# abeauvisage/uasl_motion_estimation

Hardware: AMD Instinct MI355X
Metric: frames/sec + BA iter/sec, 2000 feats x 20-keyframe window, 1/2/4/8 MI355X (higher is better)
Workload: dtype u8+f32 (MI), f64 (BA); 1 GPU; config 3: 1280x720 stereo, 2000 feats, 20-keyframe window, 11x11 MI patches; frame=KLT + MI scale LM (LM, MAX_NB_ITER 10, tolerances off) + 10 BA LM iterations, parallelism=1 independent streams (one per GPU)

## Files before the change

include/me_hip.h:

```cpp
#ifndef ME_HIP_H
#define ME_HIP_H
#include <stddef.h>
#include <stdint.h>

#ifdef __cplusplus
extern "C" {
#endif

#define ME_ABI_VERSION 4

enum {
  ME_OK = 0,
  ME_ERR_INVALID = -1,
  ME_ERR_HIP = -2,
  ME_ERR_NOMEM = -3,
  ME_ERR_UNSUPPORTED = -4,
  ME_ERR_STATE = -5,
  ME_ERR_NO_DEVICE = -6
};

typedef enum { ME_HOST = 0, ME_DEVICE = 1 } me_mem;

typedef struct me_ctx me_ctx;

// ... 124 lines not shown
  double function_tolerance;
  double gradient_tolerance;
  double parameter_tolerance;
  double initial_trust_region_radius, max_trust_region_radius, min_trust_region_radius;
  double min_lm_diagonal, max_lm_diagonal, min_relative_decrease;
  int max_num_consecutive_invalid_steps;
  int jacobi_scaling;
} me_ba_options;

typedef struct {
  int status;
  int termination;
  int iterations;
  int successful_steps;
  double initial_cost, final_cost;
} me_ba_summary;

void me_ba_default_options(me_ba_options* o);
int me_ba_solve(me_ctx* ctx, me_ba_problem* p, const me_ba_options* o, me_ba_summary* s);
int me_ba_solve_async(me_ctx* ctx, me_ba_problem* p, const me_ba_options* o);
int me_ba_wait(me_ctx* ctx, me_ba_summary* s);
int me_ba_wait_out(me_ctx* ctx, me_ba_summary* s, double* cams, double* pts);
int me_ba_reserve(me_ctx* ctx, int n_cams, int n_pts, int n_obs, int obs_dim, int fixed_frames);
typedef struct me_vo_chain_args {
  double pose[6];
  double R[9];
  double vel[6];
  int k1, k0, mode;
} me_vo_chain_args;
int me_vo_ba_chain(me_ctx* ctx, double* cams, int n_cams, double* pts, int n_pts, const int32_t* cam_src,
                   const int32_t* win_ids, const int32_t* prev_ids, int n_prev, int32_t new_from,
                   const me_vo_chain_args* a);
typedef struct me_vo_window {
  const void* stage;
  void* dev;
  size_t stage_bytes;
  int chain;
  const int32_t* cam_src;
  const int32_t* win_ids;
  const int32_t* prev_ids;
  int n_prev;
  int32_t new_from;
  me_vo_chain_args args;
  const int32_t* frame;
  const int32_t* ids;
  int first_frame;
// ... 222 lines not shown
```

uasl_motion_estimation_amd/_lib.py:

```python
from __future__ import annotations

import ctypes
import os
from ctypes import POINTER, c_double, c_float, c_int, c_int32, c_long, c_size_t, c_uint8, c_uint32, c_void_p

import numpy as np

try:
    import torch
except Exception:
    torch = None

_HERE = os.path.dirname(os.path.abspath(__file__))
LIB_PATH = os.path.join(_HERE, "libme_hip.so")

ME_OK = 0
ME_HOST = 0
ME_DEVICE = 1
ERRORS = {
    -1: "ME_ERR_INVALID",
    -2: "ME_ERR_HIP",
    -3: "ME_ERR_NOMEM",
    -4: "ME_ERR_UNSUPPORTED",
    -5: "ME_ERR_STATE",
# ... 139 lines not shown
                ("n_usable", ctypes.c_int32), ("n_inliers", ctypes.c_int32), ("steps", ctypes.c_int32),
                ("valid", ctypes.c_int32), ("R", c_double * 9), ("t_rel", c_double * 3)]


class ClaheParamsC(ctypes.Structure):
    _fields_ = [("tiles_x", c_int), ("tiles_y", c_int), ("clip_limit", c_double)]


class ToneMapParamsC(ctypes.Structure):
    _fields_ = [("lo_ppm", c_int), ("hi_ppm", c_int), ("min_span", c_int), ("alpha_q8", c_int)]


ALLREDUCE_FN = ctypes.CFUNCTYPE(c_int, POINTER(c_double), c_int, c_void_p)

EXPORTS = [
    "me_abi_version", "me_range_push", "me_range_pop", "me_device_count", "me_create", "me_destroy", "me_last_error", "me_set_stream",
    "me_get_stream", "me_set_cu_mask", "me_stream_flags", "me_cu_count", "me_synchronize", "me_malloc", "me_free", "me_memcpy_h2d", "me_memcpy_d2h", "me_memcpy_d2d",
    "me_memcpy_async", "me_host_alloc", "me_host_free", "me_hbm_copy_gbs",
    "me_timing_enable", "me_timing_read", "me_timing_reset", "me_timing_sample",
    "me_mi_scores", "me_mutual_information", "me_entropy", "me_mi_epipolar_match", "me_mi_epipolar_match_count", "me_mi_epipolar_match_lr", "me_mi_epipolar_match_lr_count", "me_vo_new_cells", "me_compare_pc", "me_ccoeff_normed", "me_quantise",
    "me_optim_default_params", "me_scale_residuals", "me_scale_normal_equations", "me_scale_jacobian",
    "me_scale_optimise", "me_scale_last_counters", "me_scale_persistent", "me_scale_state_mi", "me_scale_inliers",
    "me_ba_default_options", "me_ba_solve", "me_ba_cost", "me_ba_evaluate", "me_ba_reduced_system",
    "me_ba_solve_sharded", "me_ba_covariance", "me_ba_solve_async", "me_ba_wait", "me_ba_wait_out", "me_ba_reserve", "me_ba_window_indices",
    "me_vo_ba_chain", "me_vo_window_submit",
    "me_comm_unique_id", "me_comm_create_rccl", "me_comm_create_callback", "me_comm_destroy", "me_comm_info",
    "me_comm_allreduce", "me_comm_calibrate", "me_comm_exchange_us", "me_ba_shard_worthwhile_comm", "me_ba_solve_comm", "me_ba_shard_worthwhile", "me_ba_shard_exchange_us",
    "me_klt_default_params", "me_klt_track", "me_klt_track_fb", "me_klt_track_guided", "me_klt_track_guided_fb",
    "me_corner_default_params", "me_corner_response", "me_vo_new_corners",
    "me_rectify_map", "me_remap_tile_dims", "me_remap_q5", "me_vo_loop_set_rectify",
    "me_clahe_default_params", "me_clahe", "me_clahe_apply_rows", "me_vo_loop_set_equalise",
    "me_tonemap_default_params", "me_tonemap_state_create", "me_tonemap_state_destroy", "me_tonemap_state_reset",
    "me_tonemap_state_read", "me_tonemap16", "me_vo_loop_set_tonemap", "me_vo_loop_process16",
    "me_nms_scanline3x3",
    "me_vo_default_params", "me_vo_srand", "me_vo_rand", "me_vo_process",
    "me_mono_default_params", "me_mono_vo_process",
    "me_vo_loop_default_config", "me_vo_loop_create", "me_vo_loop_destroy", "me_vo_loop_last_error",
    "me_vo_loop_process", "me_vo_loop_finish", "me_vo_loop_results", "me_vo_loop_events", "me_vo_loop_tracks",
    "me_vo_loop_poses", "me_vo_loop_frame_obs", "me_vo_loop_frames", "me_vo_loop_stats", "me_vo_loop_set_match_lr",
    "me_motion_gate_default_params", "me_motion_gate", "me_vo_loop_set_motion_gate",
    "me_vo_loop_set_klt_predict",
    "me_kf_default_params", "me_kf_update", "me_vo_loop_set_keyframe_select", "me_vo_loop_push",
    "me_frame_pose_default_params", "me_frame_pose", "me_vo_loop_set_frame_pose", "me_vo_loop_frame_poses",
]

class MonoParamsC(ctypes.Structure):
    _fields_ = [("fu", c_double), ("fv", c_double), ("cu", c_double), ("cv", c_double), ("prob", c_double),
# ... 60 lines not shown
                                               c_void_p, c_void_p, c_int, c_int, c_int, c_int, c_int, c_double,
                                               c_float, c_void_p, c_void_p]),
        "me_mi_epipolar_match_lr": (c_int, [c_void_p, c_void_p, c_void_p, c_int, c_int, c_int, c_void_p, c_void_p,
                                            c_void_p, c_void_p, c_int, c_int, c_int, c_int, c_int, c_double, c_float,
                                            c_double, c_void_p, c_void_p, c_void_p]),
        "me_mi_epipolar_match_lr_count": (c_int, [c_void_p, c_void_p, c_void_p, c_int, c_int, c_int, c_void_p,
                                                  c_void_p, c_void_p, c_int, c_int, c_int, c_int, c_int, c_double,
                                                  c_float, c_double, c_void_p, c_void_p, c_void_p]),
        "me_vo_new_cells": (c_int, [c_void_p, c_void_p, c_void_p, c_void_p, c_int, c_int, c_int, c_float, c_int, c_int,
                                    c_double, c_double, c_int, c_int, c_int, c_void_p, c_void_p, c_void_p]),
        "me_compare_pc": (c_int, [c_void_p, c_int, c_void_p, c_void_p, c_int, c_int, c_int, c_void_p]),
        "me_ccoeff_normed": (c_int, [c_void_p, c_int, c_void_p, c_void_p, c_int, c_int, c_int, c_void_p]),
        "me_quantise": (c_int, [c_void_p, c_int, c_void_p, c_int, c_int, c_int, c_int, c_int]),
        "me_entropy": (c_int, [c_void_p, c_int, c_void_p, c_int, c_int, c_int, c_void_p]),
        "me_optim_default_params": (None, [P(OptimParamsC)]),
        "me_scale_residuals": (c_int, [c_void_p, P(ScaleStateC), c_int, P(c_double), P(c_int)]),
        "me_scale_normal_equations": (c_int, [c_void_p, P(ScaleStateC), c_int, P(c_double), P(c_double),
                                              P(c_double)]),
        "me_scale_jacobian": (c_int, [c_void_p, P(ScaleStateC), c_int, P(c_double)]),
        "me_scale_optimise": (c_int, [c_void_p, P(ScaleStateC), P(OptimParamsC), c_int, P(c_int), P(c_int),
                                      P(c_double), c_int, P(c_long)]),
        "me_scale_last_counters": (c_int, [c_void_p, P(c_long), P(c_long), P(c_long), P(c_long)]),
        "me_scale_persistent": (c_int, [c_int, c_int]),
        "me_scale_state_mi": (c_int, [c_void_p, P(ScaleStateC), P(c_double), P(c_int)]),
        "me_scale_inliers": (c_int, [c_void_p, P(ScaleStateC), c_int, c_double, P(c_int), c_int, P(c_int)]),
        "me_ba_default_options": (None, [P(BAOptionsC)]),
        "me_ba_solve": (c_int, [c_void_p, P(BAProblemC), P(BAOptionsC), P(BASummaryC)]),
        "me_ba_solve_async": (c_int, [c_void_p, P(BAProblemC), P(BAOptionsC)]),
        "me_ba_wait": (c_int, [c_void_p, P(BASummaryC)]),
        "me_ba_wait_out": (c_int, [c_void_p, P(BASummaryC), c_void_p, c_void_p]),
        "me_ba_reserve": (c_int, [c_void_p, c_int, c_int, c_int, c_int, c_int]),
        "me_vo_window_submit": (c_int, [c_void_p, P(VOWindowC), P(BAProblemC), P(BAOptionsC)]),
        "me_vo_ba_chain": (c_int, [c_void_p, c_void_p, c_int, c_void_p, c_int, c_void_p, c_void_p, c_void_p, c_int,
                                   ctypes.c_int32, P(VOChainArgsC)]),
        "me_ba_cost": (c_int, [c_void_p, P(BAProblemC), P(c_double)]),
        "me_ba_window_indices": (c_int, [c_void_p, c_void_p, c_void_p, c_int, c_int, c_void_p, c_int, c_void_p,
                                         c_void_p]),
        "me_ba_evaluate": (c_int, [c_void_p, P(BAProblemC), P(c_double), P(c_double), P(c_double)]),
        "me_ba_reduced_system": (c_int, [c_void_p, P(BAProblemC), c_double, P(c_double), P(c_double)]),
        "me_ba_covariance": (c_int, [c_void_p, P(BAProblemC), P(c_double), P(c_int)]),
        "me_ba_solve_sharded": (c_int, [c_void_p, P(BAProblemC), P(BAOptionsC), ALLREDUCE_FN, c_void_p,
                                        P(BASummaryC)]),
        "me_comm_unique_id": (c_int, [c_void_p, c_int]),
        "me_comm_create_rccl": (c_int, [c_void_p, c_int, c_int, c_void_p, P(c_void_p)]),
        "me_comm_create_callback": (c_int, [c_void_p, c_int, c_int, ALLREDUCE_FN, c_void_p, P(c_void_p)]),
        "me_comm_destroy": (None, [c_void_p]),
# ... 61 lines not shown
        "me_vo_loop_set_frame_pose": (c_int, [c_void_p, P(FramePoseParamsC)]),
        "me_vo_loop_frame_poses": (c_int, [c_void_p, P(VoFramePoseC), c_int, P(c_int)]),
        "me_tonemap_default_params": (None, [P(ToneMapParamsC)]),
        "me_tonemap_state_create": (c_int, [c_void_p, P(c_void_p)]),
        "me_tonemap_state_destroy": (c_int, [c_void_p]),
        "me_tonemap_state_reset": (c_int, [c_void_p]),
        "me_tonemap_state_read": (c_int, [c_void_p, P(ctypes.c_int32)]),
        "me_tonemap16": (c_int, [c_void_p, c_int, c_void_p, c_int, c_int, c_int, c_void_p, c_int, P(ToneMapParamsC),
                                 c_void_p]),
        "me_vo_loop_set_tonemap": (c_int, [c_void_p, P(ToneMapParamsC)]),
        "me_vo_loop_process16": (c_int, [c_void_p, c_int, c_void_p, c_void_p, c_int]),
        "me_nms_scanline3x3": (c_int, [c_void_p, c_int, c_void_p, c_int, c_int, c_void_p, c_void_p, c_int,
                                       P(c_int)]),
        "me_vo_default_params": (None, [P(VOParamsC)]),
        "me_vo_srand": (c_int, [c_void_p, ctypes.c_uint]),
        "me_vo_rand": (c_int, [c_void_p, P(c_int)]),
        "me_vo_process": (c_int, [c_void_p, c_void_p, c_int, P(c_double), P(VOParamsC), c_int, P(c_double),
                                  P(c_double), P(c_double), P(c_int), P(c_int), P(c_int)]),
        "me_mono_default_params": (None, [P(MonoParamsC)]),
        "me_mono_vo_process": (c_int, [c_void_p, c_void_p, c_void_p, c_int, P(MonoParamsC), P(c_double),
                                       P(c_double), c_void_p, P(c_int), P(c_int)]),
    }
    for name, (res, args) in sig.items():
        fn = getattr(lib, name)
        fn.restype = res
        fn.argtypes = args
    _lib = lib
    return lib


def dptr(a: np.ndarray, ctype=c_double):
    if a is None:
        return None
    assert a.flags["C_CONTIGUOUS"], "array must be C-contiguous"
    return a.ctypes.data_as(POINTER(ctype))


def vptr(a):
    if a is None:
        return None
    if isinstance(a, int):
        return c_void_p(a)
    assert a.flags["C_CONTIGUOUS"], "array must be C-contiguous"
    return c_void_p(a.ctypes.data)


def cu_split(ncu: int, front_of_16: int, mode: str | None = None):
# ... 141 lines not shown
```

uasl_motion_estimation_amd/csrc/ba.hip:

```cpp
#include <algorithm>
#include <cmath>
#include <cstdio>
#include <cstring>
#include <mutex>
#include <numeric>
#include <vector>
#include <hip/hip_ext.h>
#include "me_internal.hpp"
#include "ba_kernels.hpp"
#include "roster.hpp"
#include "solve_diag.hpp"
#include "me_device.hpp"

using me_dev::wave_sync;

using namespace ba;

namespace {

constexpr double kDblMin = 2.2250738585072014e-308;
constexpr double kDblEps = 2.220446049250313e-16;

template <int Ctrl>
__device__ __forceinline__ double dpp_f64(double x);
// ... 2727 lines not shown
  }
  __syncthreads();
  for (int p = t; p < g.npairs; p += kScanBlock) {
    int I = 0, rem = p;
    while (rem >= g.T - I) {
      rem -= g.T - I;
      ++I;
    }
    const int J = I + rem;
    int cnt = 0;
    for (int r = 0; r < g.nruns; ++r) {
      const int A = rA[r], B = rB[r];
      const int nb = B - A + 1, ns = nb + (B < g.T - 1 ? 1 : 0);
      const int ka = (I >= A && I <= B) ? I - A : (I == g.T - 1 ? nb : -1);
      const int kb = (J >= A && J <= B) ? J - A : (J == g.T - 1 ? nb : -1);
      if (ka < 0 || kb < 0) continue;
      b.tl[(long)p * g.nruns + cnt++] = r * g.npairs + ka * ns - ka * (ka - 1) / 2 + (kb - ka);
    }
    b.tcnt[p] = cnt;
    for (int q = cnt; q < g.nruns; ++q) b.tl[(long)p * g.nruns + q] = -1;
  }
}

__global__ __launch_bounds__(kBlock) void output_kernel(Geo g, Bufs b, double* cams_dst, double* pts_dst) {
  const int cur = b.st->cur;
  const long gid = (long)blockIdx.x * kBlock + threadIdx.x;
  constexpr int kStateWords = (int)(sizeof(State) / 8);
  if (gid < kStateWords) b.out[gid] = ((const double*)b.st)[gid];
  if (gid < 6 * (long)g.nc) cams_dst[gid] = b.cams[cur][gid];
  if (gid < 3 * (long)g.np) pts_dst[gid] = b.pts[cur][gid];
}

struct Plan {
  me_ctx* c = nullptr;
  Geo g;
  unsigned asm_gen = 0;
  Bufs b;
  Opts o;
  double* colnorm = nullptr;
  double* gc_raw = nullptr;
  double* Uraw = nullptr;
  double* cpart = nullptr;
  double* host = nullptr;
  State* hstate[2] = {nullptr, nullptr};
  bool dev = false;
  bool copy_out = false;
  bool reserve_only = false;
  size_t solve_lds = 0;
  size_t schur_lds = 0;
  int use_lds = 0;
  int solve_flags = 0;
  int n_enq = 0;
  bool no_fused_asm = false;
  bool fused_lin = false;
  bool full_S = false;
  int solve_cap = 0;
  me_comm* comm = nullptr;
  bool xmax_separate = false;
};

inline long rup(long x, long m) { return (x + m - 1) / m * m; }
int blocks(long n, int bs) { return (int)std::max(1L, (n + bs - 1) / bs); }

void schur_geometry(int npairs, int np, int Rpad, Geo& g) {
  const bool wide = schur_lds_bytes(kSchurPtsWide, Rpad) <= kSchurLdsCap;
  const bool split_wide = wide && npairs <= 40 && np <= 256 * kSchurPts;
  g.spts = wide ? kSchurPtsWide : npairs > 100 ? kSchurPtsSmall : kSchurPts;
  g.nsub = (int)std::max(1L, ((long)np + g.spts - 1) / g.spts);
  g.rsub = (int)std::max(1L, ((long)g.nsub + 255) / 256);
  g.rlen = g.spts * g.rsub;
  g.nruns = (int)std::max(1L, ((long)np + g.rlen - 1) / g.rlen);
  const int nt = split_wide ? 2 : npairs > 100 ? kSchurNtMax : std::min(kSchurNtMax, 4);
  g.stpw = 8 * std::min((npairs + 7) / 8, nt);
  g.sgrp = (npairs + g.stpw - 1) / g.stpw;
  g.ksplit = (g.sgrp > 1 ? (int)rup((long)g.nruns, 8) : g.nruns) * g.sgrp;
  g.sorted = npairs > 40 ? 1 : 0;
}

void ba_geometry(Geo& g, int n_cams, int fixed_frames, int n_pts) {
  g.nc = n_cams;
  g.np = n_pts;
// ... 3 lines not shown
  g.Rpad = (int)rup(g.n6 + 1, 16);
  g.T = g.Rpad / 16;
  g.Ts = (g.n6 + 1 + 15) / 16;
  g.npairs = g.T * (g.T + 1) / 2;
  schur_geometry(g.npairs, g.np, g.Rpad, g);
}

constexpr size_t kSolveLdsCap = 150 * 1024;
inline int solve_form(int Ts) {
  if (8 * (solve_small_doubles(Ts) + solve_a_doubles(Ts)) <= kSolveLdsCap) return 0;
  return Ts >= kSolveMwMinTs ? 2 : 1;
}

extern "C" int me_debug_ba_geometry(int n_cams, int fixed_frames, int n_pts, int* out) {
  if (n_cams <= 0 || n_pts < 0 || !out) return ME_ERR_INVALID;
  Geo g;
  ba_geometry(g, n_cams, fixed_frames, n_pts);
  const int v[10] = {g.spts, g.nsub, g.rsub, g.rlen, g.nruns, g.stpw, g.sgrp, g.ksplit, g.sorted, solve_form(g.Ts)};
  std::memcpy(out, v, sizeof v);
  return ME_OK;
}

int ba_drain(me_ctx* c);

int plan_build(me_ctx* c, const me_ba_problem* p, const me_ba_options* opt, Plan& P, int slot_base,
               int async = -1, me_comm* comm = nullptr) {
  if (async < 0) ME_TRY(ba_drain(c));
  ME_CHECK(c, p->n_cams > 0 && p->n_pts >= 0 && p->n_obs >= 0, "BA: bad sizes");
  ME_CHECK(c, p->n_cams <= kMaxScanCams, "BA: at most %d cameras per window", kMaxScanCams);
  ME_CHECK(c, p->obs_dim == 0 || p->obs_dim == 2 || p->obs_dim == 4, "BA: obs_dim must be 2 or 4 (Observation<M>)");
  const bool mono = p->obs_dim == 2;
  ME_CHECK(c, p->feat_var > 0 && (mono || p->baseline != 0.0), "BA: wrong calibration parameters (BundleAdjuster.h:147)");
  ME_CHECK(c, !mono || p->cam_id || p->n_obs == 0, "BA: obs_dim 2 needs cam_id (Observation::camID)");
  const double baseline = mono && p->baseline == 0 ? 0.5 : p->baseline;
  ME_CHECK(c, p->mem == ME_HOST || p->mem == ME_DEVICE, "BA: bad memory kind");
  if (p->mem == ME_HOST) {
    for (int i = 0; i < p->n_obs; ++i) {
      ME_CHECK(c, p->cam_idx[i] >= 0 && p->cam_idx[i] < p->n_cams && p->pt_idx[i] >= 0 && p->pt_idx[i] < p->n_pts,
               "BA: observation %d indexes outside the window", i);
    }
  }
  P.c = c;
  int hook = c->dbg_solve_flags;
  if ((hook & kFlagFailEveryOther) && (c->dbg_solve_count++ & 1)) hook |= kFlagSolveFail;
  P.no_fused_asm = (hook & kFlagSeparateAsm) != 0;
  P.solve_flags = hook & (kFlagAsmTimeout | kFlagSolveFail | kFlagRosterNow);
  Geo& g = P.g;
  ba_geometry(g, p->n_cams, p->fixed_frames, p->n_pts);
  g.no = p->n_obs;
  g.od = mono ? 2 : 4;
  P.comm = comm;
  P.xmax_separate = comm && comm->world == 0;
  g.xslots = comm && comm->world > 0 ? comm->world : 1;
  g.xrank = comm && comm->world > 0 ? comm->rank : 0;
  ME_CHECK(c, g.nruns <= kMaxRuns, "BA: %d Schur runs exceed %d", g.nruns, kMaxRuns);
  g.nblkp = blocks(std::max(g.np, 1), kBlock);
  ME_CHECK(c, g.npairs <= 8 * 24, "BA: %d variable cameras exceed the Schur tile budget", g.m);
  g.nblk_obs = (int)std::max(1L, rup(std::max(g.no, 1), kBlock) / kBlock);
  g.nblk_lin = (int)std::max(1L, rup(std::max(g.no, 1), lin_block(g.no)) / lin_block(g.no));
  g.nblk_pts = (int)std::max(1L, rup(std::max(g.np, 1), kPtBlock) / kPtBlock);
  P.fused_lin = schur_fused_lin(g.od, schur_nt(g.stpw), g.spts) && g.rsub == 1 && !g.sorted &&
                (g.sgrp == 1 || g.ksplit <= 128) && schur_lds_bytes(g.spts, g.Rpad) + kSchurLinLds <= kSchurLdsCap;
  g.flin = P.fused_lin ? 1 : 0;
  g.ncost = P.fused_lin ? g.nruns : g.nblk_lin;
  g.jacobi = opt->jacobi_scaling ? 1 : 0;
  g.ncu = (int)(rup(std::max(g.no, 1), kBlock) / kBlock) + g.m;
  g.nblk_step = (int)std::max(1L, rup(std::max(g.np, 1), kStepPts) / kStepPts);
  g.pstride = std::max({g.nblk_obs, g.nblk_lin, g.nblk_pts, g.nblk_step, g.ksplit});
// ... 116 lines not shown
  P.host = (double*)hp;
  if (P.reserve_only) return ME_OK;
  P.hstate[0] = (State*)((char*)hp + stage);
  P.hstate[1] = (State*)((char*)hp + stage + rup(sizeof(State), 64));
  P.dev = dev;
  hipStream_t s = c->stream;
  if (!dev) {
    char* h = (char*)hp;
    const void* src[6] = {p->cams, p->pts, p->obs, p->cam_idx, p->pt_idx, p->cam_id};
    const size_t len[6] = {8 * 6 * (size_t)g.nc, 8 * 3 * (size_t)g.np, 8 * g.od * (size_t)g.no, 4 * (size_t)g.no,
                           4 * (size_t)g.no, mono ? 4 * (size_t)g.no : 0};
    size_t off = 0;
    for (int k = 0; k < 6; ++k) {
      if (len[k]) std::memcpy(h + off, src[k], len[k]);
      off += items[k].first;
    }
    ME_HIP(c, hipMemcpyAsync(b.cams[0], hp, input_span, hipMemcpyHostToDevice, s));
  } else {
    b.obs = p->obs;
    b.cam_idx = p->cam_idx;
    b.pt_idx = p->pt_idx;
    if (mono) b.cam_id = p->cam_id;
  }
  ME_HIP(c, hipMemsetAsync(b.cnt, 0, (size_t)((char*)b.work - (char*)b.cnt) + work_bytes, s));
  P.asm_gen = 0;
  const double* cams_in = dev ? p->cams : b.cams[0];
  const double* pts_in = dev ? p->pts : b.pts[0];
  const long nthr = std::max({(long)g.nblk_obs * kBlock, (long)g.np, 6L * g.nc, 3L * g.np});
  hipLaunchKernelGGL(plan_count_kernel, dim3(blocks(nthr, kBlock)), dim3(kBlock), 4 * (size_t)g.nc, s, g, b, cams_in,
                     pts_in);
  hipLaunchKernelGGL(plan_scan_kernel, dim3(1), dim3(kScanBlock), 0, s, g, b, o);
  hipLaunchKernelGGL(plan_scatter_kernel, dim3(g.nblk_obs), dim3(kBlock), 0, s, g, b);
  hipLaunchKernelGGL(plan_segsort_kernel, dim3(blocks(std::max(g.np, 1), kSortBlock / 64)), dim3(kSortBlock), 0, s, g,
                     b);
  if (g.sorted) {
    hipLaunchKernelGGL(plan_band_kernel, dim3(g.nblkp), dim3(kBlock), 0, s, g, b);
    hipLaunchKernelGGL(plan_order_kernel, dim3(1), dim3(kScanBlock), 0, s, g, b);
  }
  ME_TRY(me_check_launch(c, "BA plan"));
  P.use_lds = solve_form(g.Ts) == 0 ? 1 : 0;
  P.solve_lds = 8 * (solve_small_doubles(g.Ts) + (P.use_lds ? solve_a_doubles(g.Ts) : 0));
  ME_CHECK(c, P.solve_lds <= kSolveLdsCap, "BA: %d variable cameras exceed the camera-solve workspace", g.m);
  P.schur_lds = schur_lds_bytes(g.spts, g.Rpad) + (P.fused_lin ? kSchurLinLds : 0);
  ME_CHECK(c, P.schur_lds <= kSchurLdsCap, "BA: %d variable cameras exceed the Schur workspace", g.m);
  if (!c->ba_lds_attr) {
    for (const void* k : {(const void*)cam_solve_kernel<0>, (const void*)cam_solve_kernel<1>, (const void*)cam_solve_kernel<2>})
      ME_HIP(c, hipFuncSetAttribute(k, hipFuncAttributeMaxDynamicSharedMemorySize, (int)kSolveLdsCap));
#define ME_SCHUR_K(D, N)                                                                                      \
  (const void*)pt_schur_kernel<D, N, 512, kSchurPts>, (const void*)pt_schur_kernel<D, N, 512, kSchurPtsWide>, \
      (const void*)pt_schur_kernel<D, N, 512, kSchurPtsSmall>
    for (const void* k : {ME_SCHUR_K(4, 2), ME_SCHUR_K(4, 3), ME_SCHUR_K(4, 4), ME_SCHUR_K(4, 5), ME_SCHUR_K(2, 2),
                          ME_SCHUR_K(2, 3), ME_SCHUR_K(2, 4), ME_SCHUR_K(2, 5)})
#undef ME_SCHUR_K
      ME_HIP(c, hipFuncSetAttribute(k, hipFuncAttributeMaxDynamicSharedMemorySize, (int)kSchurLdsCap));
    c->ba_lds_attr = 1;
  }
  if (!P.use_lds) {
    int per_cu = 0;
    ME_HIP(c, hipOccupancyMaxActiveBlocksPerMultiprocessor(&per_cu, cam_solve_kernel<2>, kSolveBlock, P.solve_lds));
    P.solve_cap = std::max(0, per_cu) * (c->cu_active > 0 ? c->cu_active : c->num_cu);
    if (P.comm && g.Ts >= kSolveMwMinTs) {
      double* d = P.b.scal;
      const double v = -(double)P.solve_cap;
      ME_HIP(c, hipMemcpyAsync(d, &v, 8, hipMemcpyHostToDevice, c->stream));
      ME_TRY(me_comm_allreduce_impl(P.comm, d, 1, ME_COMM_MAX));
      double r = 0.0;
      ME_HIP(c, hipMemcpyAsync(&r, d, 8, hipMemcpyDeviceToHost, c->stream));
      ME_HIP(c, hipStreamSynchronize(c->stream));
      P.solve_cap = (int)-r;
    }
  }
  return ME_OK;
}



#define ME_XCH(ptr, n, op) ME_TRY(me_comm_allreduce_impl(P.comm, (ptr), (long)(n), (op)))

// ... 75 lines not shown
  const int mode = P.comm ? SA_UNPACK : SA_SUM;
  if (g.m > 0)
    hipLaunchKernelGGL(s_assemble_kernel, dim3(blocks((long)g.npairs * 256, kSaElems) + 1), dim3(kBlock), 0,
                       c->stream, g, P.b, P.o, (const double*)P.gc_raw, P.full_S ? 1 : 0, mode,
                       img && !P.full_S ? P.b.Abuf : nullptr);
  else
    hipLaunchKernelGGL(lin_finalize_kernel, dim3(1), dim3(kFinBlock), 0, c->stream, g, P.b, P.o,
                       (const double*)P.gc_raw);
  return me_check_launch(c, "BA assemble");
}

int enqueue_iteration(Plan& P, bool last = false) {
  me_ctx* c = P.c;
  const Geo& g = P.g;
  hipStream_t s = c->stream;
  const bool sh = P.comm != nullptr;
  ME_TRY(enqueue_linearize(P));
  const int np0 = (g.Ts - 1) * g.Ts / 2;
  int nwk = solve_form(g.Ts) == 2 ? std::min(64, std::max(1, (np0 + kSolveBlock / 64 - 1) / (kSolveBlock / 64))) : 0;
  nwk = std::max(0, std::min(nwk, P.solve_cap - 1));
  const bool fuse = g.m > 0 && !P.full_S && !last && nwk == 0 && !P.no_fused_asm;
  const int nasm = fuse ? blocks((long)g.npairs * 256, kSolveBlock / kSaGroups) : 0;
  const bool img = !fuse && !last && g.m > 0 && !P.full_S && ME_SOLVE_IMG;
  if (!fuse) ME_TRY(enqueue_assemble(P, img));
  if (last) return me_check_launch(c, "BA iteration");
  if (g.m == 0) ME_HIP(c, hipMemsetAsync(P.b.scal + R_COUNT, 0, 8, s));
  {
    me_ktimer t(c, ME_KT_BA_SOLVE);
    const double* gc = P.gc_raw;
    const int sk = P.solve_flags | (img ? kFlagImg : 0);
    const unsigned gen = nasm > 0 ? ++P.asm_gen : 0u;
    if (P.use_lds)
      hipLaunchKernelGGL(cam_solve_kernel<0>, dim3(1 + nasm), dim3(kSolveBlock), P.solve_lds, s, g, P.b, P.o, sk, 0,
                         nasm, gc, gen);
    else if (nwk > 0)
#ifdef ME_COOP_LAUNCH
    {
      int skv = sk, nwv = nwk, z = 0;
      unsigned gv = gen;
      void* args[] = {(void*)&g, (void*)&P.b, (void*)&P.o, &skv, &nwv, &z, (void*)&gc, &gv};
      ME_HIP(c, hipLaunchCooperativeKernel((const void*)cam_solve_kernel<2>, dim3(1 + nwk), dim3(kSolveBlock), args,
                                           (unsigned)P.solve_lds, s));
    }
#else
      hipLaunchKernelGGL(cam_solve_kernel<2>, dim3(1 + nwk), dim3(kSolveBlock), P.solve_lds, s, g, P.b, P.o, sk, nwk,
                         0, gc, gen);
// ... 3 lines not shown
                         nasm, gc, gen);
  }
  {
    me_ktimer t(c, ME_KT_BA_STEP);
    if (g.od == 4)
      hipLaunchKernelGGL(pt_step_kernel<4>, dim3(g.nblk_step + 1), dim3(kStepBlock), 0, s, g, P.b, P.o, sh ? 0 : 1);
    else
      hipLaunchKernelGGL(pt_step_kernel<2>, dim3(g.nblk_step + 1), dim3(kStepBlock), 0, s, g, P.b, P.o, sh ? 0 : 1);
  }
  if (sh) {
    ME_XCH(P.b.scal + R_MODEL, 5, ME_COMM_SUM);
    hipLaunchKernelGGL(decide_kernel, dim3(1), dim3(64), 0, s, g, P.b, P.o);
  }
  return me_check_launch(c, "BA iteration");
}

int enqueue_output(Plan& P, me_ba_problem* p) {
  me_ctx* c = P.c;
  const Geo& g = P.g;
  constexpr size_t nst = sizeof(State) / 8;
  double* cams_dst = P.dev ? p->cams : P.b.out + nst;
  double* pts_dst = P.dev ? p->pts : P.b.out + nst + 6 * (size_t)g.nc;
  const long n = std::max({(long)nst, 6L * g.nc, 3L * g.np});
  hipLaunchKernelGGL(output_kernel, dim3(blocks(n, kBlock)), dim3(kBlock), 0, c->stream, g, P.b, cams_dst, pts_dst);
  ME_TRY(me_check_launch(c, "BA output"));
  const size_t bytes = 8 * (P.dev ? nst : nst + 6 * (size_t)g.nc + 3 * (size_t)g.np);
  ME_HIP(c, hipMemcpyAsync(P.host, P.b.out, bytes, hipMemcpyDeviceToHost, c->stream));
  if (P.dev && P.copy_out) {
    ME_HIP(c, hipMemcpyAsync(P.host + nst, p->cams, 8 * 6 * (size_t)g.nc, hipMemcpyDeviceToHost, c->stream));
    if (g.np)
      ME_HIP(c, hipMemcpyAsync(P.host + nst + 6 * (size_t)g.nc, p->pts, 8 * 3 * (size_t)g.np, hipMemcpyDeviceToHost,
                               c->stream));
  }
  return ME_OK;
}

int finish(Plan& P, me_ba_problem* p, me_ba_summary* sum, bool output_queued = false, hipEvent_t done = nullptr) {
  me_ctx* c = P.c;
  const Geo& g = P.g;
  constexpr size_t nst = sizeof(State) / 8;
  static_assert(sizeof(State) % 8 == 0, "State is read back as doubles");
  if (!output_queued) ME_TRY(enqueue_output(P, p));
  if (done) ME_HIP(c, hipEventSynchronize(done));
  else ME_HIP(c, hipStreamSynchronize(c->stream));
  State st;
  std::memcpy(&st, P.host, sizeof(State));
  std::memcpy(P.c->dbg, st.stamps, sizeof(st.stamps));
// ... 573 lines not shown
  pt_idx[i] = (lo < n_pts && win_ids[lo] == id) ? lo : -1;
}

extern "C" int me_ba_window_indices(me_ctx* c, const int32_t* frame, const int32_t* ids, int n_obs, int first_frame,
                                    const int32_t* win_ids, int n_pts, int32_t* cam_idx, int32_t* pt_idx) {
  if (!c) return ME_ERR_INVALID;
  ME_CHECK(c, n_obs >= 0 && n_pts >= 0, "me_ba_window_indices: bad sizes");
  if (n_obs == 0) return ME_OK;
  ME_HIP(c, hipSetDevice(c->device));
  hipLaunchKernelGGL(window_indices_kernel, dim3(blocks(n_obs, kBlock)), dim3(kBlock), 0, c->stream, frame, ids, n_obs,
                     first_frame, win_ids, n_pts, cam_idx, pt_idx);
  return me_check_launch(c, "window_indices_kernel");
}

extern "C" int me_debug_solve_flags(me_ctx* c, int flags) {
  if (!c) return ME_ERR_INVALID;
  ME_CHECK(c, (flags & ~kHookMask) == 0, "me_debug_solve_flags: 0x%x holds bits that are no test hook (accepted: 0x%x)",
           (unsigned)flags, (unsigned)kHookMask);
  c->dbg_solve_flags = flags;
  c->dbg_solve_count = 0;
  return ME_OK;
}

extern "C" int me_debug_read(me_ctx* c, long long* out, int n) {
  if (!c || n < 0 || n > 16) return ME_ERR_INVALID;
  std::memcpy(out, c->dbg, 8 * (size_t)n);
  return ME_OK;
}

#ifdef ME_CAM_TS
extern "C" int me_cam_ts(long long* out, int reset) {
  unsigned long long h[8];
  if (hipMemcpyFromSymbol(h, HIP_SYMBOL(g_cam_ts), sizeof h) != hipSuccess) return -1;
  for (int i = 0; i < 8; ++i) out[i] = (long long)h[i];
  if (reset) {
    const unsigned long long z[8] = {0, 0, 0, 0, 0, 0, 0, 0};
    if (hipMemcpyToSymbol(HIP_SYMBOL(g_cam_ts), z, sizeof z) != hipSuccess) return -1;
  }
  return 0;
}
extern "C" int me_cam_ts_unit(int unit) {
  if (unit < 0) return -1;
  return hipMemcpyToSymbol(HIP_SYMBOL(g_cam_ts_unit), &unit, sizeof unit) == hipSuccess ? 0 : -1;
}
#endif

// ... 13 lines not shown
```

uasl_motion_estimation_amd/csrc/me_internal.hpp:

```cpp
#pragma once
#include <hip/hip_runtime.h>
#include <cstdarg>
#include <cstdio>
#include <string>
#include <vector>
#include "../../include/me_hip.h"

struct me_timer_pair {
  hipEvent_t a, b;
  int kernel;
};

enum : int {
  kFlagAsmTimeout = 512,
  kFlagSolveFail = 1024,
  kFlagFailEveryOther = 2048,
  kFlagImg = 4096,
  kFlagRosterNow = 8192,
  kFlagSeparateAsm = 16384,
  kFlagMiLane = 32768,
  kHookMask = kFlagAsmTimeout | kFlagSolveFail | kFlagFailEveryOther | kFlagRosterNow | kFlagSeparateAsm | kFlagMiLane,
};

struct me_ctx {
  int device = 0;
  int num_cu = 256;
  int cu_active = 0;
  hipStream_t own_stream = nullptr;
  hipStream_t stream = nullptr;
  std::string err;
  std::vector<void*> slot_ptr;
  std::vector<size_t> slot_size;
  void* pinned = nullptr;
  size_t pinned_size = 0;
  int timing = 0;
  std::vector<me_timer_pair> pending;
  std::vector<hipEvent_t> event_pool;
  long launches[ME_KT_COUNT] = {0};
  double total_ms[ME_KT_COUNT] = {0};
  long kt_seen[ME_KT_COUNT] = {0};
  int timing_every = 1;
  hipEvent_t poll_ev[2] = {nullptr, nullptr};
  int32_t rand_st[31] = {0};
  int rand_f = 3, rand_r = 0;
  bool rand_init = false;
  long long dbg[16] = {0};
  int dbg_solve_flags = 0;
  unsigned dbg_solve_count = 0;
  void* ba_async = nullptr;
  void (*ba_async_free)(me_ctx*) = nullptr;
  void* ba_pinned[2] = {nullptr, nullptr};
  size_t ba_pinned_size[2] = {0, 0};
  int ba_lds_attr = 0;
  void* scale_mirror = nullptr;
  int scale_gen = 0;
  int scale_lm_cap = -1;
  long scale_counters[4] = {0, 0, 0, 0};
  float* mi_table[256] = {nullptr};
  bool fpose_armed = false;
  bool tonemap_armed = false;
};

struct me_comm {
  me_ctx* ctx = nullptr;
  int world = 1, rank = 0;
  void* nccl = nullptr;
  me_allreduce_fn ar = nullptr;
  void* user = nullptr;
  double xch_us[2] = {0.0, 0.0};
};
int me_comm_allreduce_impl(me_comm* m, double* buf, long n, int op);

int me_mi_table(me_ctx* ctx, int npx, const float** out);

int me_set_error(me_ctx* ctx, int code, const char* fmt, ...);

// ... 51 lines not shown
```

Measured before the change: 1376 frames/s.

## Fuse BA plan build into one LDS kernel and merge final finalize with output copy

For small BA problems (up to 64 cameras, unsorted, fitting in LDS), a single multi-workgroup plan_small_kernel replaces the memset plus the count, scan, band and order kernels. It builds per-point and per-camera observation indices in shared memory using wave ballots and prefix scans. The last iteration's assemble step is deferred into a close_kernel that runs lin_finalize alongside the output copy, removing further launches. This trades launch overhead for a more complex kernel; every workgroup recomputes the full count tables redundantly, and a legacy-plan flag keeps the old path. Debug export hooks and a planning query are also added.

```diff
diff --git a/include/me_hip.h b/include/me_hip.h
--- a/include/me_hip.h
+++ b/include/me_hip.h
@@ -170,6 +170,7 @@
 int me_ba_wait(me_ctx* ctx, me_ba_summary* s);
 int me_ba_wait_out(me_ctx* ctx, me_ba_summary* s, double* cams, double* pts);
 int me_ba_reserve(me_ctx* ctx, int n_cams, int n_pts, int n_obs, int obs_dim, int fixed_frames);
+int me_ba_plan_small(int n_obs, int n_pts, int n_cams, int fixed_frames);
 typedef struct me_vo_chain_args {
   double pose[6];
   double R[9];
diff --git a/uasl_motion_estimation_amd/_lib.py b/uasl_motion_estimation_amd/_lib.py
--- a/uasl_motion_estimation_amd/_lib.py
+++ b/uasl_motion_estimation_amd/_lib.py
@@ -185,7 +185,7 @@
     "me_optim_default_params", "me_scale_residuals", "me_scale_normal_equations", "me_scale_jacobian",
     "me_scale_optimise", "me_scale_last_counters", "me_scale_persistent", "me_scale_state_mi", "me_scale_inliers",
     "me_ba_default_options", "me_ba_solve", "me_ba_cost", "me_ba_evaluate", "me_ba_reduced_system",
-    "me_ba_solve_sharded", "me_ba_covariance", "me_ba_solve_async", "me_ba_wait", "me_ba_wait_out", "me_ba_reserve", "me_ba_window_indices",
+    "me_ba_solve_sharded", "me_ba_covariance", "me_ba_solve_async", "me_ba_wait", "me_ba_wait_out", "me_ba_reserve", "me_ba_plan_small", "me_ba_window_indices",
     "me_vo_ba_chain", "me_vo_window_submit",
     "me_comm_unique_id", "me_comm_create_rccl", "me_comm_create_callback", "me_comm_destroy", "me_comm_info",
     "me_comm_allreduce", "me_comm_calibrate", "me_comm_exchange_us", "me_ba_shard_worthwhile_comm", "me_ba_solve_comm", "me_ba_shard_worthwhile", "me_ba_shard_exchange_us",
@@ -292,6 +292,7 @@
                                       P(c_double), c_int, P(c_long)]),
         "me_scale_last_counters": (c_int, [c_void_p, P(c_long), P(c_long), P(c_long), P(c_long)]),
         "me_scale_persistent": (c_int, [c_int, c_int]),
+        "me_ba_plan_small": (c_int, [c_int, c_int, c_int, c_int]),
         "me_scale_state_mi": (c_int, [c_void_p, P(ScaleStateC), P(c_double), P(c_int)]),
         "me_scale_inliers": (c_int, [c_void_p, P(ScaleStateC), c_int, c_double, P(c_int), c_int, P(c_int)]),
         "me_ba_default_options": (None, [P(BAOptionsC)]),
@@ -399,7 +400,11 @@
                                        P(c_double), c_void_p, P(c_int), P(c_int)]),
     }
     for name, (res, args) in sig.items():
-        fn = getattr(lib, name)
+        fn = getattr(lib, name, None)
+        if fn is None and path != LIB_PATH:
+            continue
+        if fn is None:
+            raise MEError(-4, f"{path} does not export {name} (rebuild: __graft_entry__.build())")
         fn.restype = res
         fn.argtypes = args
     _lib = lib
diff --git a/uasl_motion_estimation_amd/csrc/ba.hip b/uasl_motion_estimation_amd/csrc/ba.hip
--- a/uasl_motion_estimation_amd/csrc/ba.hip
+++ b/uasl_motion_estimation_amd/csrc/ba.hip
@@ -2773,6 +2773,304 @@
   }
 }
 
+constexpr int kPlanBatch = 16, kPlanBatch2 = 4;
+constexpr int kPlanWgs = 16;
+__device__ __forceinline__ unsigned long long match_any(int key, bool valid, int nbits) {
+  unsigned long long peers = __ballot(valid);
+  for (int bit = 0; bit < nbits; ++bit) {
+    const bool set = (key >> bit) & 1;
+    const unsigned long long bal = __ballot(valid && set);
+    peers &= set ? bal : ~bal;
+  }
+  return peers;
+}
+constexpr int kPlanSmallMaxCams = 64;
+__host__ __device__ inline int plan_small_chunks(int no) { return (no + 63) / 64; }
+__host__ __device__ inline size_t plan_small_lds(int no, int np, int m) {
+  return 16 * (size_t)np + 8 + 4 * (size_t)m * (size_t)plan_small_chunks(no);
+}
+
+__global__ __launch_bounds__(kScanBlock) void plan_small_kernel(Geo g, Bufs b, Opts o, const double* cams_in,
+                                                                const double* pts_in, int nclear, int nclaim) {
+  extern __shared__ unsigned long long plan_lds[];
+  __shared__ int wsum[kScanBlock / 64];
+  __shared__ int total, ctotal;
+  __shared__ int sflag[3];
+  __shared__ int ctot[kPlanSmallMaxCams];
+  __shared__ int ufst[kPlanSmallMaxCams + 1];
+  const int t = threadIdx.x, lane = t & 63, wv = t >> 6;
+  const int nchunk = plan_small_chunks(g.no);
+  const int nwg = gridDim.x, wg = blockIdx.x;
+  const bool lead = wg == 0;
+  unsigned long long* s_mask = plan_lds;
+  int* s_cnt = (int*)(s_mask + g.np);
+  int* s_off = s_cnt + g.np;
+  int* s_tab = s_off + g.np + 1;
+  for (int j = t; j < g.np; j += kScanBlock) {
+    s_mask[j] = 0ull;
+    s_cnt[j] = 0;
+  }
+  for (int i = t; i < g.m * nchunk; i += kScanBlock) s_tab[i] = 0;
+  if (t < 3) sflag[t] = 0;
+  if (lead) {
+    for (int i = t; i < nclear; i += kScanBlock) b.cnt[i] = 0u;
+    for (int i = t; i < nclaim; i += kScanBlock) b.asm_claim[i] = 0u;
+    for (int i = t; i < g.n6; i += kScanBlock) b.csc[i] = 0.0;
+  }
+  __syncthreads();
+  if (lead) {
+    for (int j = t; j < g.np; j += kScanBlock)
+      for (int a = 0; a < 3; ++a) {
+        const double x = pts_in[3 * (long)j + a];
+        if (!(x >= g.lo[a] && x <= g.hi[a])) sflag[F_INFEASIBLE] = 1;
+      }
+    if (cams_in != b.cams[0])
+      for (int i = t; i < 6 * g.nc; i += kScanBlock) b.cams[0][i] = cams_in[i];
+    if (pts_in != b.pts[0])
+      for (int i = t; i < 3 * g.np; i += kScanBlock) b.pts[0][i] = pts_in[i];
+  }
+  for (int base = 0; base < g.no; base += kPlanBatch * kScanBlock) {
+    int ci[kPlanBatch], pi[kPlanBatch];
+#pragma unroll
+    for (int r = 0; r < kPlanBatch; ++r) {
+      const int ob = base + r * kScanBlock + t;
+      ci[r] = ob < g.no ? b.cam_idx[ob] : -1;
+      pi[r] = ob < g.no ? b.pt_idx[ob] : -1;
+    }
+#pragma unroll
+    for (int r = 0; r < kPlanBatch; ++r) {
+      const int ob = base + r * kScanBlock + t;
+      if (base + r * kScanBlock >= g.no) break;
+      bool ok = false;
+      if (ob < g.no) {
+        ok = ci[r] >= 0 && ci[r] < g.nc && pi[r] >= 0 && pi[r] < g.np;
+        if (!ok) sflag[F_BAD] = 1;
+      }
+      if (ok) {
+        atomicAdd(&s_cnt[pi[r]], 1);
+        atomicOr(&s_mask[pi[r]], 1ull << ci[r]);
+      }
+      if (ok && ci[r] >= g.nf) atomicAdd(&s_tab[(ci[r] - g.nf) * nchunk + (ob >> 6)], 1);
+    }
+  }
+  __syncthreads();
+  {
+    const int chunk = (g.np + kScanBlock - 1) / kScanBlock;
+    const int beg = min(g.np, t * chunk), end = min(g.np, beg + chunk);
+    int s = 0;
+    for (int j = beg; j < end; ++j) s += s_cnt[j];
+    int x = s;
+    for (int off = 1; off < 64; off <<= 1) {
+      const int y = __shfl_up(x, off, 64);
+      if (lane >= off) x += y;
+    }
+    if (lane == 63) wsum[wv] = x;
+    __syncthreads();
+    if (t == 0) {
+      int acc = 0;
+      for (int k = 0; k < kScanBlock / 64; ++k) {
+        const int v = wsum[k];
+        wsum[k] = acc;
+        acc += v;
+      }
+      total = acc;
+    }
+    __syncthreads();
+    int run = wsum[wv] + x - s;
+    for (int j = beg; j < end; ++j) {
+      const int cj = s_cnt[j];
+      if (lead) b.p_off[j] = run;
+      s_off[j] = run;
+      run += cj;
+      const bool plain = cj == __builtin_popcountll(s_mask[j]);
+      s_cnt[j] = plain ? -1 : 0;
+      if (!plain) sflag[2] = 1;
+    }
+    if (t == 0) {
+      if (lead) b.p_off[g.np] = total;
+      s_off[g.np] = total;
+    }
+  }
+  const int bchunk = (nchunk + 63) / 64;
+  for (int c = wv; c < g.m; c += kScanBlock / 64) {
+    const int k0 = min(nchunk, lane * bchunk), k1 = min(nchunk, k0 + bchunk);
+    int cs = 0;
+    for (int k = k0; k < k1; ++k) cs += s_tab[c * nchunk + k];
+    int cx = cs;
+    for (int off = 1; off < 64; off <<= 1) {
+      const int y = __shfl_up(cx, off, 64);
+      if (lane >= off) cx += y;
+    }
+    int r = cx - cs;
+    for (int k = k0; k < k1; ++k) {
+      const int v = s_tab[c * nchunk + k];
+      s_tab[c * nchunk + k] = r;
+      r += v;
+    }
+    if (lane == 63) ctot[c] = cx;
+  }
+  __syncthreads();
+  if (t == 0) {
+    int acc = 0, units = 0;
+    for (int c = 0; c < g.m; ++c) {
+      if (lead) b.c_off[c] = acc;
+      const int v = ctot[c];
+      ctot[c] = acc;
+      acc += v;
+      ufst[c] = units;
+      units += max(1, (v + kBlock - 1) / kBlock);
+    }
+    if (lead) b.c_off[g.m] = acc;
+    ctotal = acc;
+    ufst[g.m] = units;
+  }
+  __syncthreads();
+  for (int c = wv; lead && c < g.m; c += kScanBlock / 64) {
+    const int cbeg = ctot[c], cend = c + 1 < g.m ? ctot[c + 1] : ctotal;
+    const int first = ufst[c], count = ufst[c + 1] - first;
+    for (int k = lane; k < count; k += 64) {
+      int* e = b.cunit + (long)kCuStride * (first + k);
+      e[CU_CAM] = c;
+      e[CU_BEG] = cbeg + k * kBlock;
+      e[CU_END] = min(cend, cbeg + (k + 1) * kBlock);
+      e[CU_COUNT] = count;
+      e[CU_FIRST] = first;
+    }
+  }
+  for (int u = ufst[g.m] + t; lead && u < (g.ncu + 7) / 8 * 8; u += kScanBlock)
+    b.cunit[(long)kCuStride * u + CU_CAM] = -1;
+  if (lead && t == 0) {
+    State* st = b.st;
+    st->cur = 0;
+    st->need_lin = 1;
+    st->done = 0;
+    st->termination = 1;
+    st->iterations = st->successful = st->invalid_count = 0;
+    st->fail = st->scaled = st->accepted = st->final_pass = st->spin_err = 0;
+    st->bad_input = sflag[F_BAD];
+    st->infeasible = sflag[F_INFEASIBLE];
+    st->radius = o.initial_radius;
+    st->decrease = 2.0;
+    st->x_cost = st->cand_cost = st->model_change = st->initial_cost = 0.0;
+    st->cam_step2 = st->cam_xn2 = st->cam_model = st->last_q = 0.0;
+    for (int k = 0; k < 16; ++k) st->stamps[k] = 0;
+    st->stamps[14] = ufst[g.m];
+    if (st->bad_input || st->infeasible) {
+      st->done = 1;
+      st->termination = 2;
+    }
+  }
+  if (sflag[F_BAD]) return;
+  int nbits = 0;
+  while ((1 << nbits) < g.m) ++nbits;
+  const int nround = (g.no + kScanBlock - 1) / kScanBlock;
+  for (int rd0 = wg; rd0 < nround; rd0 += kPlanBatch2 * nwg) {
+    int ci[kPlanBatch2], pi[kPlanBatch2];
+#pragma unroll
+    for (int r = 0; r < kPlanBatch2; ++r) {
+      const long ob = ((long)rd0 + (long)r * nwg) * kScanBlock + t;
+      ci[r] = ob < g.no ? b.cam_idx[ob] : -1;
+      pi[r] = ob < g.no ? b.pt_idx[ob] : -1;
+    }
+#pragma unroll
+    for (int r = 0; r < kPlanBatch2; ++r) {
+      if (rd0 + r * nwg >= nround) break;
+      const int ob = (rd0 + r * nwg) * kScanBlock + t;
+      const int vc = ci[r] >= g.nf ? ci[r] - g.nf : -1;
+      const unsigned long long peers = match_any(vc, vc >= 0, nbits);
+      if (ob < g.no) {
+        int slot = -1;
+        if (vc >= 0) {
+          slot = ctot[vc] + s_tab[vc * nchunk + (ob >> 6)] + __builtin_popcountll(peers & ((1ull << lane) - 1ull));
+          b.c_obs[slot] = ob;
+        }
+        b.cpos[ob] = slot;
+        const int p = pi[r];
+        if (s_cnt[p] < 0) {
+          const int q = s_off[p] + __builtin_popcountll(s_mask[p] & ((1ull << ci[r]) - 1ull));
+          b.p_obs[q] = ob;
+          b.pos[ob] = q;
+          b.p_cam[q] = ci[r] - g.nf;
+          b.dup[ob] = 0;
+        }
+      }
+    }
+  }
+  if (!sflag[2]) return;
+  for (int base = 0; base < g.no; base += kPlanBatch * kScanBlock) {
+    int pi[kPlanBatch];
+#pragma unroll
+    for (int r = 0; r < kPlanBatch; ++r) {
+      const int ob = base + r * kScanBlock + t;
+      pi[r] = ob < g.no ? b.pt_idx[ob] : -1;
+    }
+#pragma unroll
+    for (int r = 0; r < kPlanBatch; ++r) {
+      const int ob = base + r * kScanBlock + t;
+      const int p = pi[r];
+      if (ob < g.no && p % nwg == wg && s_cnt[p] >= 0) b.tmp_obs[s_off[p] + atomicAdd(&s_cnt[p], 1)] = ob;
+    }
+  }
+  __syncthreads();
+  for (int j = wv; j < g.np; j += kScanBlock / 64) {
+    if (j % nwg != wg || s_cnt[j] < 0) continue;
+    const int beg = s_off[j], k = s_off[j + 1] - beg;
+    auto key_of = [&](int ob) { return ((unsigned long long)(unsigned)b.cam_idx[ob] << 32) | (unsigned)ob; };
+    if (k <= 64) {
+      const int ob = lane < k ? b.tmp_obs[beg + lane] : 0;
+      const unsigned long long key = lane < k ? key_of(ob) : ~0ull;
+      int rank = 0, same = 0;
+      for (int l = 0; l < k; ++l) {
+        const unsigned long long kl = __shfl(key, l, 64);
+        rank += kl < key;
+        same += (kl >> 32) == (key >> 32);
+      }
+      if (lane < k) {
+        const int q = beg + rank;
+        b.p_obs[q] = ob;
+        b.pos[ob] = q;
+        b.p_cam[q] = (int)(key >> 32) - g.nf;
+        b.dup[ob] = same > 1 ? 1 : 0;
+      }
+      continue;
+    }
+    for (int e = lane; e < k; e += 64) {
+      const int ob = b.tmp_obs[beg + e];
+      const unsigned long long key = key_of(ob);
+      int rank = 0, same = 0;
+      for (int l = 0; l < k; ++l) {
+        const unsigned long long kl = key_of(b.tmp_obs[beg + l]);
+        rank += kl < key;
+        same += (kl >> 32) == (key >> 32);
+      }
+      const int q = beg + rank;
+      b.p_obs[q] = ob;
+      b.pos[ob] = q;
+      b.p_cam[q] = (int)(key >> 32) - g.nf;
+      b.dup[ob] = same > 1 ? 1 : 0;
+    }
+  }
+}
+
+__global__ __launch_bounds__(kBlock) void close_kernel(Geo g, Bufs b, Opts o, const double* gc_raw, double* cams_dst,
+                                                       double* pts_dst) {
+  static_assert(kBlock == kFinBlock, "the finalize block runs with the copy block size");
+  if (blockIdx.x == gridDim.x - 1) {
+    __shared__ double lds[16];
+    if (threadIdx.x < 2) b.ssync[threadIdx.x] = 0u;
+    lin_finalize_body(g, b, o, gc_raw, lds);
+    __syncthreads();
+    constexpr int kStateWords = (int)(sizeof(State) / 8);
+    static_assert(kStateWords <= kBlock, "one thread per State word");
+    if (threadIdx.x < kStateWords) b.out[threadIdx.x] = ((const double*)b.st)[threadIdx.x];
+    return;
+  }
+  const int cur = b.st->cur;
+  const long gid = (long)blockIdx.x * kBlock + threadIdx.x;
+  if (gid < 6 * (long)g.nc) cams_dst[gid] = b.cams[cur][gid];
+  if (gid < 3 * (long)g.np) pts_dst[gid] = b.pts[cur][gid];
+}
+
 __global__ __launch_bounds__(kBlock) void output_kernel(Geo g, Bufs b, double* cams_dst, double* pts_dst) {
   const int cur = b.st->cur;
   const long gid = (long)blockIdx.x * kBlock + threadIdx.x;
@@ -2808,6 +3106,9 @@
   int solve_cap = 0;
   me_comm* comm = nullptr;
   bool xmax_separate = false;
+  bool legacy_plan = false;
+  bool small_plan = false;
+  bool close_pending = false;
 };
 
 inline long rup(long x, long m) { return (x + m - 1) / m * m; }
@@ -2857,6 +3158,17 @@
 }
 
 int ba_drain(me_ctx* c);
+
+bool plan_small_fits(const Geo& g) {
+  return g.nc <= kPlanSmallMaxCams && !g.sorted && plan_small_lds(g.no, g.np, g.m) + 1024 <= kSchurLdsCap;
+}
+
+struct DebugPlan {
+  int no = 0, np = 0, m = 0, ncu8 = 0, small = 0;
+  const void* arr[9] = {nullptr};
+};
+DebugPlan* debug_plan(me_ctx* c) { return (DebugPlan*)c->dbg_plan; }
+static_assert(sizeof(DebugPlan) <= sizeof(me_ctx::dbg_plan), "me_ctx holds the last plan's description");
 
 int plan_build(me_ctx* c, const me_ba_problem* p, const me_ba_options* opt, Plan& P, int slot_base,
                int async = -1, me_comm* comm = nullptr) {
@@ -2879,6 +3191,7 @@
   int hook = c->dbg_solve_flags;
   if ((hook & kFlagFailEveryOther) && (c->dbg_solve_count++ & 1)) hook |= kFlagSolveFail;
   P.no_fused_asm = (hook & kFlagSeparateAsm) != 0;
+  P.legacy_plan = (hook & kFlagLegacyPlan) != 0;
   P.solve_flags = hook & (kFlagAsmTimeout | kFlagSolveFail | kFlagRosterNow);
   Geo& g = P.g;
   ba_geometry(g, p->n_cams, p->fixed_frames, p->n_pts);
@@ -3041,10 +3354,25 @@
     b.pt_idx = p->pt_idx;
     if (mono) b.cam_id = p->cam_id;
   }
-  ME_HIP(c, hipMemsetAsync(b.cnt, 0, (size_t)((char*)b.work - (char*)b.cnt) + work_bytes, s));
-  P.asm_gen = 0;
   const double* cams_in = dev ? p->cams : b.cams[0];
   const double* pts_in = dev ? p->pts : b.pts[0];
+  P.asm_gen = 0;
+  P.small_plan = !P.legacy_plan && plan_small_fits(g);
+  DebugPlan* D = debug_plan(c);
+  *D = DebugPlan{g.no, g.np, g.m, (int)rup(g.ncu, 8), P.small_plan ? 1 : 0,
+                 {b.p_off, b.p_obs, b.pos, b.p_cam, b.dup, b.c_off, b.c_obs, b.cpos, b.cunit}};
+  if (P.small_plan) {
+    if (!(c->ba_lds_attr & 2)) {
+      ME_HIP(c, hipFuncSetAttribute((const void*)plan_small_kernel, hipFuncAttributeMaxDynamicSharedMemorySize,
+                                    (int)kSchurLdsCap));
+      c->ba_lds_attr |= 2;
+    }
+    const int nclaim = blocks((long)g.npairs * 256, kSolveBlock / kSaGroups);
+    const int nwg = std::min(kPlanWgs, blocks(g.no, kScanBlock));
+    hipLaunchKernelGGL(plan_small_kernel, dim3(nwg), dim3(kScanBlock), plan_small_lds(g.no, g.np, g.m), s, g, b, o,
+                       cams_in, pts_in, g.m + 1 + 3 + 2, nclaim);
+  } else {
+  ME_HIP(c, hipMemsetAsync(b.cnt, 0, (size_t)((char*)b.work - (char*)b.cnt) + work_bytes, s));
   const long nthr = std::max({(long)g.nblk_obs * kBlock, (long)g.np, 6L * g.nc, 3L * g.np});
   hipLaunchKernelGGL(plan_count_kernel, dim3(blocks(nthr, kBlock)), dim3(kBlock), 4 * (size_t)g.nc, s, g, b, cams_in,
                      pts_in);
@@ -3056,13 +3384,14 @@
     hipLaunchKernelGGL(plan_band_kernel, dim3(g.nblkp), dim3(kBlock), 0, s, g, b);
     hipLaunchKernelGGL(plan_order_kernel, dim3(1), dim3(kScanBlock), 0, s, g, b);
   }
+  }
   ME_TRY(me_check_launch(c, "BA plan"));
   P.use_lds = solve_form(g.Ts) == 0 ? 1 : 0;
   P.solve_lds = 8 * (solve_small_doubles(g.Ts) + (P.use_lds ? solve_a_doubles(g.Ts) : 0));
   ME_CHECK(c, P.solve_lds <= kSolveLdsCap, "BA: %d variable cameras exceed the camera-solve workspace", g.m);
   P.schur_lds = schur_lds_bytes(g.spts, g.Rpad) + (P.fused_lin ? kSchurLinLds : 0);
   ME_CHECK(c, P.schur_lds <= kSchurLdsCap, "BA: %d variable cameras exceed the Schur workspace", g.m);
-  if (!c->ba_lds_attr) {
+  if (!(c->ba_lds_attr & 1)) {
     for (const void* k : {(const void*)cam_solve_kernel<0>, (const void*)cam_solve_kernel<1>, (const void*)cam_solve_kernel<2>})
       ME_HIP(c, hipFuncSetAttribute(k, hipFuncAttributeMaxDynamicSharedMemorySize, (int)kSolveLdsCap));
 #define ME_SCHUR_K(D, N)                                                                                      \
@@ -3072,7 +3401,7 @@
                           ME_SCHUR_K(2, 3), ME_SCHUR_K(2, 4), ME_SCHUR_K(2, 5)})
 #undef ME_SCHUR_K
       ME_HIP(c, hipFuncSetAttribute(k, hipFuncAttributeMaxDynamicSharedMemorySize, (int)kSchurLdsCap));
-    c->ba_lds_attr = 1;
+    c->ba_lds_attr |= 1;
   }
   if (!P.use_lds) {
     int per_cu = 0;
@@ -3194,6 +3523,10 @@
   const bool fuse = g.m > 0 && !P.full_S && !last && nwk == 0 && !P.no_fused_asm;
   const int nasm = fuse ? blocks((long)g.npairs * 256, kSolveBlock / kSaGroups) : 0;
   const bool img = !fuse && !last && g.m > 0 && !P.full_S && ME_SOLVE_IMG;
+  if (last && g.m > 0 && !sh && !P.full_S && !P.legacy_plan) {
+    P.close_pending = true;
+    return me_check_launch(c, "BA iteration");
+  }
   if (!fuse) ME_TRY(enqueue_assemble(P, img));
   if (last) return me_check_launch(c, "BA iteration");
   if (g.m == 0) ME_HIP(c, hipMemsetAsync(P.b.scal + R_COUNT, 0, 8, s));
@@ -3243,7 +3576,13 @@
   double* cams_dst = P.dev ? p->cams : P.b.out + nst;
   double* pts_dst = P.dev ? p->pts : P.b.out + nst + 6 * (size_t)g.nc;
   const long n = std::max({(long)nst, 6L * g.nc, 3L * g.np});
-  hipLaunchKernelGGL(output_kernel, dim3(blocks(n, kBlock)), dim3(kBlock), 0, c->stream, g, P.b, cams_dst, pts_dst);
+  if (P.close_pending) {
+    P.close_pending = false;
+    hipLaunchKernelGGL(close_kernel, dim3(blocks(std::max(6L * g.nc, 3L * g.np), kBlock) + 1), dim3(kBlock), 0, c->stream,
+                       g, P.b, P.o, (const double*)P.gc_raw, cams_dst, pts_dst);
+  } else {
+    hipLaunchKernelGGL(output_kernel, dim3(blocks(n, kBlock)), dim3(kBlock), 0, c->stream, g, P.b, cams_dst, pts_dst);
+  }
   ME_TRY(me_check_launch(c, "BA output"));
   const size_t bytes = 8 * (P.dev ? nst : nst + 6 * (size_t)g.nc + 3 * (size_t)g.np);
   ME_HIP(c, hipMemcpyAsync(P.host, P.b.out, bytes, hipMemcpyDeviceToHost, c->stream));
@@ -3863,6 +4202,38 @@
   return ME_OK;
 }
 
+extern "C" int me_ba_plan_small(int n_obs, int n_pts, int n_cams, int fixed_frames) {
+  if (n_cams <= 0 || n_pts < 0 || n_obs < 0) return ME_ERR_INVALID;
+  Geo g;
+  ba_geometry(g, n_cams, fixed_frames, n_pts);
+  g.no = n_obs;
+  return plan_small_fits(g) ? 1 : 0;
+}
+
+extern "C" int me_debug_ba_plan(me_ctx* c, int which, int32_t* out, int n) {
+  if (!c || !out || n < 0 || which < 0 || which > 9) return ME_ERR_INVALID;
+  const DebugPlan* D = debug_plan(c);
+  if (which == 9) {
+    if (n > 0) out[0] = D->small;
+    return 1;
+  }
+  const long len[9] = {D->np + 1L, D->no, D->no, D->no, D->no, D->m + 1L, D->no, D->no, (long)kCuStride * D->ncu8};
+  ME_CHECK(c, D->arr[which] != nullptr, "me_debug_ba_plan: no plan was built on this context");
+  const long cnt = std::min<long>(n, len[which]);
+  ME_HIP(c, hipSetDevice(c->device));
+  ME_HIP(c, hipStreamSynchronize(c->stream));
+  if (cnt > 0) {
+    if (which == 4) {
+      std::vector<uint8_t> h((size_t)cnt);
+      ME_HIP(c, hipMemcpy(h.data(), D->arr[which], (size_t)cnt, hipMemcpyDeviceToHost));
+      for (long i = 0; i < cnt; ++i) out[i] = h[(size_t)i];
+    } else {
+      ME_HIP(c, hipMemcpy(out, D->arr[which], 4 * (size_t)cnt, hipMemcpyDeviceToHost));
+    }
+  }
+  return (int)len[which];
+}
+
 extern "C" int me_debug_read(me_ctx* c, long long* out, int n) {
   if (!c || n < 0 || n > 16) return ME_ERR_INVALID;
   std::memcpy(out, c->dbg, 8 * (size_t)n);
diff --git a/uasl_motion_estimation_amd/csrc/me_internal.hpp b/uasl_motion_estimation_amd/csrc/me_internal.hpp
--- a/uasl_motion_estimation_amd/csrc/me_internal.hpp
+++ b/uasl_motion_estimation_amd/csrc/me_internal.hpp
@@ -19,7 +19,9 @@
   kFlagRosterNow = 8192,
   kFlagSeparateAsm = 16384,
   kFlagMiLane = 32768,
-  kHookMask = kFlagAsmTimeout | kFlagSolveFail | kFlagFailEveryOther | kFlagRosterNow | kFlagSeparateAsm | kFlagMiLane,
+  kFlagLegacyPlan = 65536,
+  kHookMask = kFlagAsmTimeout | kFlagSolveFail | kFlagFailEveryOther | kFlagRosterNow | kFlagSeparateAsm | kFlagMiLane |
+              kFlagLegacyPlan,
 };
 
 struct me_ctx {
@@ -52,6 +54,7 @@
   void* ba_pinned[2] = {nullptr, nullptr};
   size_t ba_pinned_size[2] = {0, 0};
   int ba_lds_attr = 0;
+  long long dbg_plan[16] = {0};
   void* scale_mirror = nullptr;
   int scale_gen = 0;
   int scale_lm_cap = -1;
```

Result: no change. 1384 frames/s (median of 6 runs) (+0.6%).
